# nhcha6/embodied-object-detection

Hardware: NVIDIA B200
Metric: memory write+read frames/sec (480x640, C=256) (higher is better)
Workload: dtype f32

## Files before the change

### embodied-object-detection_b200/csrc/write_mean.cu

```cuda
#include <cuda.h>
#include <stdlib.h>

#include "eod_common.cuh"
#include "tmap_cache.cuh"

namespace {

constexpr int TILE_PX = 32;

constexpr int kCountSpan = 4;

__global__ void __launch_bounds__(256) frame_count_kernel(const int32_t *__restrict__ idx, const uint8_t *__restrict__ samp,
                                                          const int32_t *__restrict__ active, int HW, int64_t n_cells,
                                                          uint32_t *__restrict__ frame_cnt, int32_t *__restrict__ slot_of_cell,
                                                          int32_t *__restrict__ slot_cell, int32_t *__restrict__ n_slots, int S)
{
    const int e = blockIdx.y;
    if (active && __ldg(active + e) <= 0) return;
    const unsigned lane = threadIdx.x & 31;
    int cellv[kCountSpan];
    bool sv[kCountSpan], validv[kCountSpan];
#pragma unroll
    for (int it = 0; it < kCountSpan; ++it) {
        const int p = (blockIdx.x * kCountSpan + it) * (int)blockDim.x + (int)threadIdx.x;
// ... 130 lines not shown
                r[h] = i < n ? (size_t)(vb * 4 + s_row[i]) * C : 0;
#pragma unroll
                for (int k = 0; k < 4; ++k)
                    if (i < n && (int)lane + 32 * k < c4) x[h][k] = reinterpret_cast<const float4 *>(sums + r[h])[lane + 32 * k];
            }
#pragma unroll
            for (int h = 0; h < 2; ++h) {
                if (i0 + 8 * h >= n) continue;
                uint2 *dst_row = reinterpret_cast<uint2 *>(norm16 + r[h]);
#pragma unroll
                for (int k = 0; k < 4; ++k) {
                    if ((int)lane + 32 * k >= c4) continue;
                    float4 y = x[h][k];
                    if (wn[h] > 1.0f) { y.x = __fdiv_rn(y.x, wn[h]); y.y = __fdiv_rn(y.y, wn[h]); y.z = __fdiv_rn(y.z, wn[h]); y.w = __fdiv_rn(y.w, wn[h]); }
                    __half2 a = __floats2half2_rn(y.x, y.y), b2 = __floats2half2_rn(y.z, y.w);
                    uint2 raw;
                    raw.x = *reinterpret_cast<uint32_t *>(&a);
                    raw.y = *reinterpret_cast<uint32_t *>(&b2);
                    dst_row[lane + 32 * k] = raw;
                }
                for (int k = lane + 128; k < c4; k += 32) {
                    float4 y = reinterpret_cast<const float4 *>(sums + r[h])[k];
                    if (wn[h] > 1.0f) { y.x = __fdiv_rn(y.x, wn[h]); y.y = __fdiv_rn(y.y, wn[h]); y.z = __fdiv_rn(y.z, wn[h]); y.w = __fdiv_rn(y.w, wn[h]); }
                    __half2 a = __floats2half2_rn(y.x, y.y), b2 = __floats2half2_rn(y.z, y.w);
                    uint2 raw;
                    raw.x = *reinterpret_cast<uint32_t *>(&a);
                    raw.y = *reinterpret_cast<uint32_t *>(&b2);
                    dst_row[k] = raw;
                }
            }
        }
        __syncthreads();
    }
}

__global__ void __launch_bounds__(256) expand_counts_kernel(const int32_t *__restrict__ idx, const uint32_t *__restrict__ frame_cnt,
                                                            int HW, int64_t n_cells, float *__restrict__ pix_n)
{
    const int e = blockIdx.y;
    const int p = blockIdx.x * blockDim.x + threadIdx.x;
    if (p >= HW) return;
    const size_t g = (size_t)e * HW + p;
    const uint32_t n = __ldg(frame_cnt + (size_t)e * n_cells + __ldg(idx + g)) & 0x7fffffffu;
    pix_n[g] = n ? __frcp_rn((float)n) : 0.f;
}

__global__ void __launch_bounds__(256) expand_counts_vec4_kernel(const int32_t *__restrict__ idx, const uint32_t *__restrict__ frame_cnt,
                                                                 int HW, int64_t n_cells, float *__restrict__ pix_n)
{
    const int e = blockIdx.y;
    const int p = (blockIdx.x * blockDim.x + threadIdx.x) * 4;
    if (p >= HW) return;
    const size_t g = (size_t)e * HW + p;
    const int4 c = __ldg(reinterpret_cast<const int4 *>(idx + g));
    const uint32_t *cnt = frame_cnt + (size_t)e * n_cells;
    const uint32_t n0 = __ldg(cnt + c.x) & 0x7fffffffu, n1 = __ldg(cnt + c.y) & 0x7fffffffu, n2 = __ldg(cnt + c.z) & 0x7fffffffu,
                   n3 = __ldg(cnt + c.w) & 0x7fffffffu;
    *reinterpret_cast<float4 *>(pix_n + g) = make_float4(n0 ? __frcp_rn((float)n0) : 0.f, n1 ? __frcp_rn((float)n1) : 0.f,
                                                         n2 ? __frcp_rn((float)n2) : 0.f, n3 ? __frcp_rn((float)n3) : 0.f);
}

__global__ void __launch_bounds__(1024) sample_mask_kernel(const uint8_t *__restrict__ observed, int HW, int stride,
                                                           uint8_t *__restrict__ samp, int32_t *__restrict__ n_sampled)
{
    __shared__ int s_warp[32];
    __shared__ int s_carry;
    const int e = blockIdx.x;
    const uint8_t *obs = observed + (size_t)e * HW;
    uint8_t *out = samp + (size_t)e * HW;
    const unsigned lane = threadIdx.x & 31, warp = threadIdx.x >> 5;
    if (threadIdx.x == 0) s_carry = 0;
    __syncthreads();
    int sampled_total = 0;
    for (int base = 0; base < HW; base += 1024) {
        const int p = base + threadIdx.x;
        const bool o = p < HW && obs[p] != 0;
        const unsigned bal = __ballot_sync(0xffffffffu, o);
        const int within = __popc(bal & ((1u << lane) - 1u));
        if (lane == 0) s_warp[warp] = __popc(bal);
        __syncthreads();
        int pre = 0;
        for (int w = 0; w < (int)warp; ++w) pre += s_warp[w];
        const int carry = s_carry;
        const int rank = carry + pre + within;
        const bool s = o && (rank % stride == 0);
        if (p < HW) out[p] = s ? 1 : 0;
        sampled_total += s ? 1 : 0;
        __syncthreads();
        if (threadIdx.x == 1023) s_carry = carry + pre + __popc(bal);
        __syncthreads();
    }
    if (n_sampled) {
        for (int o = 16; o > 0; o >>= 1) sampled_total += __shfl_xor_sync(0xffffffffu, sampled_total, o);
        if (lane == 0) s_warp[warp] = sampled_total;
        __syncthreads();
        if (threadIdx.x == 0) {
            int t = 0;
            for (int w = 0; w < 32; ++w) t += s_warp[w];
            n_sampled[e] = t;
        }
    }
}

__global__ void __launch_bounds__(1024) sample_mask_vec_kernel(const uint8_t *__restrict__ observed, int HW, int stride,
                                                               uint8_t *__restrict__ samp, int32_t *__restrict__ n_sampled)
{
    __shared__ int s_warp[2][32];
    const int e = blockIdx.x;
    const uint4 *obs = reinterpret_cast<const uint4 *>(observed + (size_t)e * HW);
    uint4 *out = reinterpret_cast<uint4 *>(samp + (size_t)e * HW);
    const unsigned lane = threadIdx.x & 31, warp = threadIdx.x >> 5;
    const int n_vec = HW >> 4;
    int carry = 0, sampled_total = 0, buf = 0;
    for (int base = 0; base < n_vec; base += 1024, buf ^= 1) {
        const int vi = base + threadIdx.x;
        uint4 q = vi < n_vec ? __ldg(obs + vi) : make_uint4(0u, 0u, 0u, 0u);
        uint32_t w[4] = {q.x, q.y, q.z, q.w};
        int cnt = 0;
#pragma unroll
        for (int k = 0; k < 4; ++k) {
            uint32_t nz = w[k] | (w[k] >> 4);
            nz |= nz >> 2;
            nz |= nz >> 1;
            w[k] = nz & 0x01010101u;
            cnt += __popc(w[k]);
        }
        int incl = cnt;
#pragma unroll
        for (int o = 1; o < 32; o <<= 1) {
            const int up = __shfl_up_sync(0xffffffffu, incl, o);
            if ((int)lane >= o) incl += up;
        }
        if (lane == 31) s_warp[buf][warp] = incl;
        __syncthreads();
        int pre = 0, total = 0;
#pragma unroll 8
        for (int x = 0; x < 32; ++x) {
            const int t = s_warp[buf][x];
            pre += x < (int)warp ? t : 0;
            total += t;
        }
        int r = (carry + pre + incl - cnt) % stride;
        carry += total;
#pragma unroll
        for (int k = 0; k < 4; ++k) {
            uint32_t o4 = 0;
#pragma unroll
            for (int b = 0; b < 4; ++b)
                if ((w[k] >> (8 * b)) & 1u) {
                    if (r == 0) { o4 |= 1u << (8 * b); ++sampled_total; }
                    if (++r == stride) r = 0;
                }
            w[k] = o4;
        }
        if (vi < n_vec) out[vi] = make_uint4(w[0], w[1], w[2], w[3]);
    }
    if (n_sampled) {
        for (int o = 16; o > 0; o >>= 1) sampled_total += __shfl_xor_sync(0xffffffffu, sampled_total, o);
        __syncthreads();
        if (lane == 0) s_warp[0][warp] = sampled_total;
        __syncthreads();
        if (threadIdx.x == 0) {
            int t = 0;
            for (int x = 0; x < 32; ++x) t += s_warp[0][x];
            n_sampled[e] = t;
        }
    }
}

__global__ void __launch_bounds__(256) box_to_image_kernel(const float *__restrict__ box_features, const uint8_t *__restrict__ masks,
                                                           int K, int C, int HW, float *__restrict__ image_features,
                                                           uint8_t *__restrict__ observed)
{
    extern __shared__ float s_feat[];
    constexpr int CH = 16;
    const int c0 = blockIdx.y * CH;
    for (int i = threadIdx.x; i < K * CH; i += blockDim.x) {
        const int k = i / CH, c = i % CH;
        s_feat[i] = (c0 + c < C) ? box_features[(size_t)k * C + c0 + c] : 0.f;
    }
    __syncthreads();
    const int p = blockIdx.x * blockDim.x + threadIdx.x;
    if (p >= HW) return;
    float acc[CH];
#pragma unroll
    for (int c = 0; c < CH; ++c) acc[c] = 0.f;
    int n = 0;
    for (int k = 0; k < K; ++k) {
        if (__ldg(masks + (size_t)k * HW + p)) {
            ++n;
#pragma unroll
            for (int c = 0; c < CH; ++c) acc[c] = __fadd_rn(acc[c], s_feat[k * CH + c]);
        }
    }
    const float fn = (float)n;
#pragma unroll
    for (int c = 0; c < CH; ++c)
        if (c0 + c < C) image_features[(size_t)(c0 + c) * HW + p] = n ? __fdiv_rn(acc[c], fn) : 0.f;
    if (blockIdx.y == 0 && observed) observed[p] = n ? 1 : 0;
}


__device__ __forceinline__ int swz(int c, int p) { return c * TILE_PX + ((((p >> 2) ^ (c & 7)) << 2) | (p & 3)); }

template <int C>
__device__ __forceinline__ void flush_runs(const float *tile, const int *s_cells, unsigned heads, unsigned samps, int pvalid,
                                           const uint32_t *__restrict__ frame_cnt_e, float *__restrict__ sums_e, int tid)
{
    constexpr int G = C / 4;
    const int nruns = __popc(heads);
    for (int item = tid; item < nruns * G; item += C) {
        const int r = item / G, g = item - r * G;
        const int p0 = __fns(heads, 0, r + 1);
        const unsigned above = heads & ~((2u << p0) - 1u);
        const int p1 = above ? (__ffs(above) - 1) : pvalid;
        const unsigned run = ((p1 >= 32) ? 0xffffffffu : ((1u << p1) - 1u)) & ~((1u << p0) - 1u);
        if (!(samps & run)) continue;
        const int cell = s_cells[p0];
        const float n = (float)(__ldg(frame_cnt_e + cell) & 0x7fffffffu);
        const int c = 4 * g;
        const float a = tile[swz(c, r)], b = tile[swz(c + 1, r)], d = tile[swz(c + 2, r)], f = tile[swz(c + 3, r)];
        red_add_v4(sums_e + (size_t)cell * C + c, __fdiv_rn(a, n), __fdiv_rn(b, n), __fdiv_rn(d, n), __fdiv_rn(f, n));
    }
}

__device__ __forceinline__ void accumulate_runs(float *tile, int c, unsigned heads, unsigned samps)
{
    float acc = 0.f;
    int r = 0;
    const float4 *row = reinterpret_cast<const float4 *>(tile + c * TILE_PX);
#pragma unroll
    for (int j = 0; j < 8; ++j) {
        const float4 v = row[j ^ (c & 7)];
        const float vv[4] = {v.x, v.y, v.z, v.w};
#pragma unroll
        for (int k = 0; k < 4; ++k) {
            const int p = 4 * j + k;
            if (p > 0 && ((heads >> p) & 1u)) {
                tile[swz(c, r)] = acc;
                ++r;
                acc = 0.f;
            }
            if ((samps >> p) & 1u) acc = __fadd_rn(acc, vv[k]);
        }
    }
    tile[swz(c, r)] = acc;
}

__device__ __forceinline__ void tile_masks(const int *s_cells, const uint8_t *s_samp, bool has_samp, int pvalid, unsigned lane,
                                           unsigned &heads, unsigned &samps)
{
    const bool valid = (int)lane < pvalid;
    const int cell = valid ? s_cells[lane] : -1;
    const int prev = __shfl_up_sync(0xffffffffu, cell, 1);
    heads = __ballot_sync(0xffffffffu, valid && (lane == 0 || prev != cell));
    samps = __ballot_sync(0xffffffffu, valid && (has_samp ? s_samp[lane] != 0 : true));
}

template <int C>
__global__ void __launch_bounds__(C) write_mean_chw_ldg_kernel(const float *__restrict__ feat, const int32_t *__restrict__ idx,
                                                               const uint8_t *__restrict__ samp, const uint32_t *__restrict__ frame_cnt,
                                                               const int32_t *__restrict__ active, int HW, int64_t n_cells, int tiles_per_ep, int n_tiles,
                                                               float *__restrict__ sums)
{
    extern __shared__ __align__(1024) unsigned char smem_raw[];
    float *tile = reinterpret_cast<float *>(smem_raw);
    int *s_cells = reinterpret_cast<int *>(tile + C * TILE_PX);
    uint8_t *s_samp = reinterpret_cast<uint8_t *>(s_cells + TILE_PX);
    const int tid = threadIdx.x, lane = tid & 31, warp = tid >> 5;
    constexpr int NW = C / 32;

    for (int t = blockIdx.x; t < n_tiles; t += gridDim.x) {
        const int e = t / tiles_per_ep, p0 = (t - e * tiles_per_ep) * TILE_PX;
        if (active && __ldg(active + e) <= 0) continue;
        const int pvalid = min(TILE_PX, HW - p0);
        const float *feat_e = feat + (size_t)e * C * HW;
#pragma unroll 4
        for (int c = warp; c < C; c += NW)
            tile[swz(c, lane)] = lane < pvalid ? __ldg(feat_e + (size_t)c * HW + p0 + lane) : 0.f;
        if (tid < TILE_PX) {
            s_cells[tid] = tid < pvalid ? __ldg(idx + (size_t)e * HW + p0 + tid) : -1;
            s_samp[tid] = (samp && tid < pvalid) ? __ldg(samp + (size_t)e * HW + p0 + tid) : 1;
        }
        __syncthreads();
        unsigned heads, samps;
        tile_masks(s_cells, s_samp, samp != nullptr, pvalid, lane, heads, samps);
        accumulate_runs(tile, tid, heads, samps);
        __syncthreads();
        flush_runs<C>(tile, s_cells, heads, samps, pvalid, frame_cnt + (size_t)e * n_cells, sums + (size_t)e * n_cells * C, tid);
        __syncthreads();
    }
}


template <int C>
struct TmaCfg {
    static constexpr int kChanBlk = C < 256 ? C : 256;
    static constexpr int kBlocks = C / kChanBlk;
    static constexpr int kJ = kChanBlk / 32;
    static constexpr int kUnitBytes = kChanBlk * TILE_PX * 4;
    static constexpr int kStages = (192 * 1024) / kUnitBytes;
    static constexpr int kThreads = 32 * (kStages + 1);
    static constexpr int kAuxCells = 0, kAuxSamp = 128, kAuxPixN = 256, kAuxUnit = 384, kAuxBytes = 512;
    static constexpr int kSmemBytes = kStages * (kUnitBytes + kAuxBytes) + 1024  + 256 ;
    static_assert(C % kChanBlk == 0 && kChanBlk % 128 == 0, "C must be 128 or a multiple of 256");
    static_assert(kSmemBytes <= 232448, "exceeds 227 KB of shared memory");
};

__device__ __forceinline__ uint64_t make_evict_first_policy()
{
    uint64_t pol;
    asm volatile("createpolicy.fractional.L2::evict_first.b64 %0, 1.0;" : "=l"(pol));
    return pol;
}

__device__ __forceinline__ void tma_load_3d_hint(uint32_t dst, const void *tmap, int x, int y, int z, uint32_t bar, uint64_t pol)
{
    asm volatile(
        "cp.async.bulk.tensor.3d.shared::cluster.global.mbarrier::complete_tx::bytes.L2::cache_hint [%0], [%1, {%2, %3, %4}], [%5], %6;" ::"r"(dst),
        "l"(tmap), "r"(x), "r"(y), "r"(z), "r"(bar), "l"(pol)
        : "memory");
}
__device__ __forceinline__ void bulk_load_1d_s(uint32_t dst, const void *src, uint32_t bytes, uint32_t bar)
{
    asm volatile("cp.async.bulk.shared::cluster.global.mbarrier::complete_tx::bytes [%0], [%1], %2, [%3];" ::"r"(dst), "l"(src), "r"(bytes), "r"(bar)
                 : "memory");
}
__device__ __forceinline__ void mbar_wait_s(uint32_t bar, uint32_t parity)
{
    asm volatile(
        "{\n\t"
        ".reg .pred p;\n\t"
        "WAIT_LOOP_S:\n\t"
        "mbarrier.try_wait.parity.shared::cta.b64 p, [%0], %1;\n\t"
        "@p bra DONE_S;\n\t"
        "bra WAIT_LOOP_S;\n\t"
        "DONE_S:\n\t"
        "}" ::"r"(bar),
        "r"(parity)
        : "memory");
}
__device__ __forceinline__ void mbar_wait_hint(uint32_t bar, uint32_t parity, uint32_t hint_ns)
{
    if (hint_ns == 0) { mbar_wait_s(bar, parity); return; }
    asm volatile(
        "{\n\t"
        ".reg .pred p;\n\t"
        "WAIT_LOOP_H:\n\t"
        "mbarrier.try_wait.parity.shared::cta.b64 p, [%0], %1, %2;\n\t"
        "@p bra DONE_H;\n\t"
        "bra WAIT_LOOP_H;\n\t"
        "DONE_H:\n\t"
        "}" ::"r"(bar),
        "r"(parity), "r"(hint_ns)
        : "memory");
}
__device__ __forceinline__ float4 lds128(uint32_t addr)
{
    float4 v;
    asm volatile("ld.shared.v4.f32 {%0, %1, %2, %3}, [%4];" : "=f"(v.x), "=f"(v.y), "=f"(v.z), "=f"(v.w) : "r"(addr));
    return v;
}
__device__ __forceinline__ uint32_t lds32(uint32_t addr)
{
    uint32_t v;
    asm volatile("ld.shared.u32 %0, [%1];" : "=r"(v) : "r"(addr));
    return v;
}
__device__ __forceinline__ void sts64(uint32_t addr, uint32_t a, uint32_t b)
{
    asm volatile("st.shared.v2.u32 [%0], {%1, %2};" ::"r"(addr), "r"(a), "r"(b) : "memory");
}
__device__ __forceinline__ uint32_t lds8(uint32_t addr)
{
    uint32_t v;
    asm volatile("ld.shared.u8 %0, [%1];" : "=r"(v) : "r"(addr));
    return v;
}

struct DetArgs {
    const int32_t *tile_off;
    float *partials;
    int32_t *run_cell;
    int32_t *status;
    int cap;
};

template <int C, bool kDry, bool kPixN, bool kDet>
__global__ void __launch_bounds__(TmaCfg<C>::kThreads, 1)
write_mean_chw_tma_kernel(const __grid_constant__ CUtensorMap tmap, const int32_t *__restrict__ idx, const uint8_t *__restrict__ samp,
                          const uint32_t *__restrict__ frame_cnt, const float *__restrict__ pix_n, const int32_t *__restrict__ active, int HW,
                          int64_t n_cells, int tiles_per_ep, int n_tiles, int group, float *__restrict__ sums, const DetArgs det,
                          int *__restrict__ work, int chunk, uint32_t wait_hint, int n_stages, int no_red)
{
    using Cfg = TmaCfg<C>;
    extern __shared__ unsigned char smem_dyn[];
    const uint32_t base = (smem_u32(smem_dyn) + 1023u) & ~1023u;
    const uint32_t aux0 = base + Cfg::kStages * Cfg::kUnitBytes;
    const uint32_t full0 = aux0 + Cfg::kStages * Cfg::kAuxBytes, empty0 = full0 + 8 * Cfg::kStages;

    const int tid = threadIdx.x;
    const int warp = tid >> 5;
    const unsigned lane = tid & 31;
    const bool has_samp = samp != nullptr;
    if (tid == 0) {
        for (int s = 0; s < Cfg::kStages; ++s) {
            asm volatile("mbarrier.init.shared::cta.b64 [%0], %1;" ::"r"(full0 + 8 * s), "r"(1));
            asm volatile("mbarrier.init.shared::cta.b64 [%0], %1;" ::"r"(empty0 + 8 * s), "r"(1));
        }
        mbar_fence_init();
        fence_proxy_async();
    }
    __syncthreads();

    const int G = (int)gridDim.x, b = (int)blockIdx.x;
    const int n_groups = n_tiles / group;
    const int units_per_group = group * Cfg::kBlocks;

    if (warp == Cfg::kStages) {
        if (lane == 0) {
            const uint64_t pol = make_evict_first_policy();
            const uint32_t tx = Cfg::kUnitBytes + TILE_PX * 4 + (has_samp ? TILE_PX : 0) + (kPixN ? TILE_PX * 4 : 0);
            int stage = 0;
            uint32_t phase = 0;
            int c = b;
            int c_next = work ? G + atomicAdd(work, 1) : c + G;
            while (c * chunk < n_groups) {
              const int c_next2 = work ? G + atomicAdd(work, 1) : c_next + G;
              const int q_end = min(n_groups, (c + 1) * chunk);
              for (int q = c * chunk; q < q_end; ++q) {
                for (int k = 0; k < units_per_group; ++k) {
                    const int cb = k / group, t = group * q + (k - cb * group);
                    const int e = t / tiles_per_ep, p0 = (t - e * tiles_per_ep) * TILE_PX;
                    const uint32_t fullb = full0 + 8 * stage, aux = aux0 + stage * Cfg::kAuxBytes;
                    mbar_wait_hint(empty0 + 8 * stage, phase ^ 1, wait_hint);
                    const bool idle = active && __ldg(active + e) <= 0;
                    sts64(aux + Cfg::kAuxUnit, (uint32_t)t, (uint32_t)cb | (idle ? 0x100u : 0u));
                    if (idle) {
                        asm volatile("mbarrier.arrive.shared::cta.b64 _, [%0];" ::"r"(fullb) : "memory");
                    } else {
                        asm volatile("mbarrier.arrive.expect_tx.shared::cta.b64 _, [%0], %1;" ::"r"(fullb), "r"(tx) : "memory");
                        tma_load_3d_hint(base + stage * Cfg::kUnitBytes, &tmap, p0, cb * Cfg::kChanBlk, e, fullb, pol);
                        bulk_load_1d_s(aux + Cfg::kAuxCells, idx + (size_t)e * HW + p0, TILE_PX * 4, fullb);
                        if (has_samp) bulk_load_1d_s(aux + Cfg::kAuxSamp, samp + (size_t)e * HW + p0, TILE_PX, fullb);
                        if (kPixN) bulk_load_1d_s(aux + Cfg::kAuxPixN, pix_n + (size_t)e * HW + p0, TILE_PX * 4, fullb);
                    }
                    if (++stage == n_stages) { stage = 0; phase ^= 1; }
                }
              }
              c = c_next;
              c_next = c_next2;
            }
            for (int s = 0; s < n_stages; ++s) {
                mbar_wait_hint(empty0 + 8 * stage, phase ^ 1, wait_hint);
                sts64(aux0 + stage * Cfg::kAuxBytes + Cfg::kAuxUnit, 0xffffffffu, 0u);
                asm volatile("mbarrier.arrive.shared::cta.b64 _, [%0];" ::"r"(full0 + 8 * stage) : "memory");
                if (++stage == n_stages) { stage = 0; phase ^= 1; }
            }
            if (work) {
                __threadfence();
                if (atomicAdd(work + 1, 1) == G - 1) {
                    work[0] = 0;
                    work[1] = 0;
                    __threadfence();
                }
            }
        }
        return;
    }

    if (warp >= n_stages) return;
    constexpr int kJ = Cfg::kJ;
    const uint32_t tile = base + warp * Cfg::kUnitBytes + lane * (TILE_PX * 4);
    const uint32_t aux = aux0 + warp * Cfg::kAuxBytes;
    const uint32_t fullb = full0 + 8 * warp, emptyb = empty0 + 8 * warp;
    const uint32_t sw = lane & 7;
    for (uint32_t phase = 0;; phase ^= 1) {
        mbar_wait_hint(fullb, phase, wait_hint);
        const int t = (int)lds32(aux + Cfg::kAuxUnit);
        if (t < 0) break;
        const uint32_t cbw = lds32(aux + Cfg::kAuxUnit + 4);
        const int cb = (int)(cbw & 0xffu);
        const bool idle = (cbw & 0x100u) != 0;
        int run_pos = kDet ? __ldg(det.tile_off + t) : 0;
        if (!kDry && !idle) {
            const int e = t / tiles_per_ep;
            const int cell = (int)lds32(aux + Cfg::kAuxCells + 4 * lane);
            const int prev = __shfl_up_sync(0xffffffffu, cell, 1);
            const unsigned grp = kDet ? 0u : __match_any_sync(0xffffffffu, cell);
            unsigned heads = __ballot_sync(0xffffffffu, kDet ? (lane == 0 || prev != cell) : ((unsigned)(__ffs(grp) - 1) == lane));
            const unsigned samps = has_samp ? __ballot_sync(0xffffffffu, lds8(aux + Cfg::kAuxSamp + lane) != 0) : 0xffffffffu;
            const float my_inv = kPixN ? __uint_as_float(lds32(aux + Cfg::kAuxPixN + 4 * lane)) : 0.f;
            float *dst = sums + ((size_t)e * n_cells) * C + cb * Cfg::kChanBlk + lane;
            const uint32_t *cnt_e = frame_cnt + (size_t)e * n_cells;

            while (heads) {
                const int p0 = __ffs(heads) - 1;
                heads &= heads - 1;
                unsigned m;
                if (kDet) {
                    const int p1 = heads ? (__ffs(heads) - 1) : TILE_PX;
                    m = samps & (0xffffffffu >> (32 - p1)) & (0xffffffffu << p0);
                } else {
                    m = samps & __shfl_sync(0xffffffffu, grp, p0);
                }
                if (m == 0) continue;
                float acc[kJ];
#pragma unroll
                for (int k = 0; k < kJ; ++k) acc[k] = 0.f;
                const int j1 = (31 - __clz(m)) >> 2;
#pragma unroll 1
                for (int j = (__ffs(m) - 1) >> 2; j <= j1; ++j) {
                    const unsigned mj = (m >> (4 * j)) & 15u;
                    if (mj == 0) continue;
                    const uint32_t a = tile + (((uint32_t)j ^ sw) << 4);
                    float4 v[kJ];
#pragma unroll
                    for (int k = 0; k < kJ; ++k) v[k] = lds128(a + k * 32 * TILE_PX * 4);
                    if (mj == 15u) {
#pragma unroll
                        for (int k = 0; k < kJ; ++k) acc[k] = __fadd_rn(__fadd_rn(__fadd_rn(__fadd_rn(acc[k], v[k].x), v[k].y), v[k].z), v[k].w);
                    } else {
                        if (mj & 1u) {
#pragma unroll
                            for (int k = 0; k < kJ; ++k) acc[k] = __fadd_rn(acc[k], v[k].x);
                        }
                        if (mj & 2u) {
#pragma unroll
                            for (int k = 0; k < kJ; ++k) acc[k] = __fadd_rn(acc[k], v[k].y);
                        }
                        if (mj & 4u) {
#pragma unroll
                            for (int k = 0; k < kJ; ++k) acc[k] = __fadd_rn(acc[k], v[k].z);
                        }
                        if (mj & 8u) {
#pragma unroll
                            for (int k = 0; k < kJ; ++k) acc[k] = __fadd_rn(acc[k], v[k].w);
                        }
                    }
                }
                const int rc = __shfl_sync(0xffffffffu, cell, p0);
                if (kDet) {
                    const int pos = run_pos++;
                    if (pos < det.cap) {
                        float *d = det.partials + ((size_t)e * det.cap + pos) * C + cb * Cfg::kChanBlk + lane;
#pragma unroll
                        for (int k = 0; k < kJ; ++k) d[32 * k] = acc[k];
                        if (cb == 0 && lane == 0) det.run_cell[(size_t)e * det.cap + pos] = rc;
                        continue;
                    }
                    if (cb == 0 && lane == 0) *det.status = 1;
                }
                float inv = __shfl_sync(0xffffffffu, my_inv, p0);
                if (!kPixN) inv = __frcp_rn((float)(__ldg(cnt_e + rc) & 0x7fffffffu));
                float *d = dst + (size_t)rc * C;
                if (no_red) continue;
#pragma unroll
                for (int k = 0; k < kJ; ++k) red_add_f32(d + 32 * k, __fmul_rn(acc[k], inv));
            }
        }
        __syncwarp();
        if (lane == 0) asm volatile("mbarrier.arrive.shared::cta.b64 _, [%0];" ::"r"(emptyb) : "memory");
    }
}

enum { FEAT_F32 = 0, FEAT_BF16 = 1, FEAT_F16 = 2 };
template <int F> struct FeatRaw { uint2 q; };
template <> struct FeatRaw<FEAT_F32> { float4 q; };
template <int F>
__device__ __forceinline__ FeatRaw<F> load_feat_raw(const void *row, int k)
{
    FeatRaw<F> r;
    if constexpr (F == FEAT_F32) r.q = ldg_stream_f4(reinterpret_cast<const float *>(row) + 4 * k);
    else asm volatile("ld.global.nc.L1::no_allocate.v2.u32 {%0, %1}, [%2];" : "=r"(r.q.x), "=r"(r.q.y) : "l"(reinterpret_cast<const uint2 *>(row) + k));
    return r;
}
template <int F>
__device__ __forceinline__ float4 widen_feat(const FeatRaw<F> &r)
{
    if constexpr (F == FEAT_F32) return r.q;
    else if constexpr (F == FEAT_BF16)
        return make_float4(__uint_as_float(r.q.x << 16), __uint_as_float(r.q.x & 0xffff0000u), __uint_as_float(r.q.y << 16), __uint_as_float(r.q.y & 0xffff0000u));
    else {
        const float2 a = __half22float2(*reinterpret_cast<const __half2 *>(&r.q.x)), b = __half22float2(*reinterpret_cast<const __half2 *>(&r.q.y));
        return make_float4(a.x, a.y, b.x, b.y);
    }
}

template <int C, int F>
__global__ void __launch_bounds__(256, 3) write_mean_hwc_kernel(const void *__restrict__ feat, const int32_t *__restrict__ idx,
                                                             const uint8_t *__restrict__ samp, const uint32_t *__restrict__ frame_cnt,
                                                             const int32_t *__restrict__ active, int HW, int64_t n_cells, int strips_per_ep,
                                                             int n_strips, float *__restrict__ sums)
{
    constexpr int V = C / 128;
    const unsigned lane = threadIdx.x & 31;
    const int warps_total = gridDim.x * (blockDim.x >> 5);
    for (int s = blockIdx.x * (blockDim.x >> 5) + (threadIdx.x >> 5); s < n_strips; s += warps_total) {
        const int e = s / strips_per_ep, p0 = (s - e * strips_per_ep) * TILE_PX;
        if (active && __ldg(active + e) <= 0) continue;
        const int pvalid = min(TILE_PX, HW - p0);
        const size_t pix0 = (size_t)e * HW + p0;
        const int my_cell = (int)lane < pvalid ? __ldg(idx + pix0 + lane) : -1;
        const bool my_s = (int)lane < pvalid && (samp ? __ldg(samp + pix0 + lane) != 0 : true);
        const unsigned samps = __ballot_sync(0xffffffffu, my_s);
        const uint32_t *cnt_e = frame_cnt + (size_t)e * n_cells;
        float *sums_e = sums + (size_t)e * n_cells * C;
        const unsigned grp = __match_any_sync(0xffffffffu, my_cell);
        unsigned leaders = __ballot_sync(0xffffffffu, (int)lane < pvalid && (unsigned)(__ffs(grp) - 1) == lane);
        constexpr int PB = (F == FEAT_F32 ? 8 : 16) / V > 0 ? (F == FEAT_F32 ? 8 : 16) / V : 1;
        while (leaders) {
            const int lead = __ffs(leaders) - 1;
            leaders &= leaders - 1;
            unsigned rem = __shfl_sync(0xffffffffu, grp, lead) & samps;
            if (rem == 0u) continue;
            const int cell = __shfl_sync(0xffffffffu, my_cell, lead);
            float4 acc[V];
#pragma unroll
            for (int v = 0; v < V; ++v) acc[v] = make_float4(0.f, 0.f, 0.f, 0.f);
#pragma unroll 1
            while (rem) {
                FeatRaw<F> raw[PB][V];
                unsigned batch = rem;
                int nb = 0;
#pragma unroll
                for (int b = 0; b < PB; ++b) {
                    if (batch) {
                        const int p = __ffs(batch) - 1;
                        batch &= batch - 1;
                        ++nb;
                        const char *row = reinterpret_cast<const char *>(feat) + (pix0 + p) * C * (F == FEAT_F32 ? 4 : 2);
#pragma unroll
                        for (int v = 0; v < V; ++v) raw[b][v] = load_feat_raw<F>(row, v * 32 + (int)lane);
                    }
                }
                rem = batch;
#pragma unroll
                for (int b = 0; b < PB; ++b) {
                    if (b < nb) {
#pragma unroll
                        for (int v = 0; v < V; ++v) {
                            const float4 f = widen_feat<F>(raw[b][v]);
                            acc[v].x = __fadd_rn(acc[v].x, f.x); acc[v].y = __fadd_rn(acc[v].y, f.y);
                            acc[v].z = __fadd_rn(acc[v].z, f.z); acc[v].w = __fadd_rn(acc[v].w, f.w);
                        }
                    }
                }
            }
            const float n = (float)(__ldg(cnt_e + cell) & 0x7fffffffu);
#pragma unroll
            for (int v = 0; v < V; ++v)
                red_add_v4(sums_e + (size_t)cell * C + v * 128 + 4 * lane, __fdiv_rn(acc[v].x, n), __fdiv_rn(acc[v].y, n), __fdiv_rn(acc[v].z, n),
                           __fdiv_rn(acc[v].w, n));
        }
    }
}

typedef CUresult (*PFN_encodeTiled)(CUtensorMap *, CUtensorMapDataType, cuuint32_t, void *, const cuuint64_t *, const cuuint64_t *,
                                    const cuuint32_t *, const cuuint32_t *, CUtensorMapInterleave, CUtensorMapSwizzle,
                                    CUtensorMapL2promotion, CUtensorMapFloatOOBfill);

PFN_encodeTiled get_encode_fn()
{
    static PFN_encodeTiled fn = nullptr;
    if (!fn) {
        void *p = nullptr;
        cudaDriverEntryPointQueryResult qres;
        if (cudaGetDriverEntryPoint("cuTensorMapEncodeTiled", &p, cudaEnableDefault, &qres) == cudaSuccess && qres == cudaDriverEntryPointSuccess)
            fn = reinterpret_cast<PFN_encodeTiled>(p);
    }
    return fn;
}

template <int C, bool kDry, bool kPixN, bool kDet = false>
int launch_tma_kernel(const CUtensorMap &tmap, const int32_t *idx, const uint8_t *samp, const uint32_t *frame_cnt, const float *pix_n,
                      const int32_t *active, int E, int HW, int64_t n_cells, float *sums, cudaStream_t st, const DetArgs det = DetArgs{})
{
    using Cfg = TmaCfg<C>;
    static unsigned long long attr_done = 0ull;
    if (int rc_attr = eod_ensure_dyn_smem(write_mean_chw_tma_kernel<C, kDry, kPixN, kDet>, Cfg::kSmemBytes, &attr_done, "eod_write_mean[tma]")) return rc_attr;
    const int tiles_per_ep = HW / TILE_PX, n_tiles = tiles_per_ep * E;
    static const int group_env = [] { const char *v = getenv("EOD_TMA_TILE_GROUP"); return v ? atoi(v) : 2; }();
    int group = (group_env == 1 || group_env == 2 || group_env == 4 || group_env == 8) ? group_env : 2;
    while (group > 1 && n_tiles % group) group >>= 1;
    const int n_groups = n_tiles / group;
    const int grid = n_groups < eod_num_sms() ? n_groups : eod_num_sms();
    static const int static_env = [] { const char *v = getenv("EOD_TMA_STATIC_TILES"); return v ? atoi(v) : 0; }();
    cudaStreamCaptureStatus cap = cudaStreamCaptureStatusNone;
    const bool capturing = cudaStreamIsCapturing(st, &cap) != cudaSuccess || cap != cudaStreamCaptureStatusNone;
    int *work = (static_env || capturing) ? nullptr : eod_work_tickets();
    static const int chunk_env = [] { const char *v = getenv("EOD_TMA_CHUNK"); return v ? atoi(v) : 8; }();
    static const int hint_env = [] { const char *v = getenv("EOD_TMA_WAIT_HINT_NS"); return v ? atoi(v) : 0; }();
    static const int stages_env = [] { const char *v = getenv("EOD_TMA_STAGES"); const int n = v ? atoi(v) : Cfg::kStages; return n >= 2 && n <= Cfg::kStages ? n : Cfg::kStages; }();
    static const int nored_env = [] { const char *v = getenv("EOD_TMA_NO_RED"); return v ? atoi(v) : 0; }();
    const int chunk = work ? (chunk_env > 0 ? chunk_env : 8) : 1;
    write_mean_chw_tma_kernel<C, kDry, kPixN, kDet><<<grid, Cfg::kThreads, Cfg::kSmemBytes, st>>>(tmap, idx, samp, frame_cnt, pix_n, active, HW, n_cells, tiles_per_ep, n_tiles, group, sums, det, work, chunk, (uint32_t)hint_env, stages_env, nored_env);
    return eod_check_launch("eod_write_mean[tma]");
}

template <int C>
int make_feature_tmap(const float *feat, int E, int HW, CUtensorMap *tmap)
{
    using Cfg = TmaCfg<C>;
    PFN_encodeTiled enc = get_encode_fn();
    EOD_REQUIRE(enc, EOD_ERR_LAUNCH, "eod_write_mean: cuTensorMapEncodeTiled entry point unavailable");
    const cuuint64_t gdim[3] = {(cuuint64_t)HW, (cuuint64_t)C, (cuuint64_t)E};
    const cuuint64_t gstr[2] = {(cuuint64_t)HW * 4, (cuuint64_t)HW * C * 4};
    const cuuint32_t box[3] = {TILE_PX, (cuuint32_t)Cfg::kChanBlk, 1};
    static const int promo_env = [] { const char *v = getenv("EOD_TMA_L2_PROMOTION"); return v ? atoi(v) : 256; }();
    const CUtensorMapL2promotion promo = promo_env == 0 ? CU_TENSOR_MAP_L2_PROMOTION_NONE
                                         : (promo_env == 128 ? CU_TENSOR_MAP_L2_PROMOTION_L2_128B : CU_TENSOR_MAP_L2_PROMOTION_L2_256B);
    const CUresult r = eod_encode_tmap_cached(enc, tmap, CU_TENSOR_MAP_DATA_TYPE_FLOAT32, 3, feat, gdim, gstr, box, promo);
    EOD_REQUIRE(r == CUDA_SUCCESS, EOD_ERR_LAUNCH, "eod_write_mean: cuTensorMapEncodeTiled failed (%d)", (int)r);
    return EOD_OK;
}

template <int C, bool kDry>
int launch_tma(const float *feat, const int32_t *idx, const uint8_t *samp, const uint32_t *frame_cnt, const float *pix_n, const int32_t *active,
               int E, int HW, int64_t n_cells, float *sums, cudaStream_t st)
{
    CUtensorMap tmap;
    const int rc = make_feature_tmap<C>(feat, E, HW, &tmap);
    if (rc) return rc;
    if (pix_n) return launch_tma_kernel<C, kDry, true>(tmap, idx, samp, frame_cnt, pix_n, active, E, HW, n_cells, sums, st);
    return launch_tma_kernel<C, kDry, false>(tmap, idx, samp, frame_cnt, nullptr, active, E, HW, n_cells, sums, st);
}

__device__ __forceinline__ void det_tile_masks(const int32_t *idx, const uint8_t *samp, size_t g0, unsigned lane, int &cell, unsigned &heads,
                                               unsigned &samps)
{
    cell = __ldg(idx + g0 + lane);
    const int prev = __shfl_up_sync(0xffffffffu, cell, 1);
    heads = __ballot_sync(0xffffffffu, lane == 0 || prev != cell);
    samps = samp ? __ballot_sync(0xffffffffu, __ldg(samp + g0 + lane) != 0) : 0xffffffffu;
}

__device__ __forceinline__ bool det_run_sampled(unsigned heads, unsigned samps, int p0)
{
    const unsigned above = heads & ~((2u << p0) - 1u);
    const int p1 = above ? (__ffs(above) - 1) : 32;
    const unsigned m = samps & (0xffffffffu >> (32 - p1)) & (0xffffffffu << p0);
    return m != 0;
}

__global__ void __launch_bounds__(256) det_tile_runs_kernel(const int32_t *__restrict__ idx, const uint8_t *__restrict__ samp, int HW,
                                                            int tiles_per_ep, int32_t *__restrict__ tile_off, int32_t *__restrict__ n_list,
                                                            int32_t *__restrict__ chunk_rows, int32_t *__restrict__ n_long)
{
    const int e = blockIdx.y, tile = blockIdx.x * 8 + (threadIdx.x >> 5);
    const unsigned lane = threadIdx.x & 31;
    if (blockIdx.x == 0 && threadIdx.x == 0) {
        n_list[e] = 0;
        chunk_rows[e] = 0;
        n_long[e] = 0;
    }
    if (tile >= tiles_per_ep) return;
    int cell;
    unsigned heads, samps;
    det_tile_masks(idx, samp, (size_t)e * HW + (size_t)tile * 32, lane, cell, heads, samps);
    const bool mine = ((heads >> lane) & 1u) && det_run_sampled(heads, samps, lane);
    const unsigned runs = __ballot_sync(0xffffffffu, mine);
    if (lane == 0) tile_off[(size_t)e * tiles_per_ep + tile] = __popc(runs);
}

__device__ void det_block_exclusive_scan(const int32_t *in, int32_t *out, int n, int32_t *total_out)
{
    __shared__ int s_warp[32];
    __shared__ int s_carry;
    const unsigned lane = threadIdx.x & 31, warp = threadIdx.x >> 5;
    if (threadIdx.x == 0) s_carry = 0;
    __syncthreads();
    for (int base = 0; base < n; base += 1024) {
        const int i = base + threadIdx.x;
        const int v = i < n ? in[i] : 0;
        int x = v;
#pragma unroll
        for (int o = 1; o < 32; o <<= 1) {
            const int y = __shfl_up_sync(0xffffffffu, x, o);
            if ((int)lane >= o) x += y;
        }
        if (lane == 31) s_warp[warp] = x;
        __syncthreads();
        if (warp == 0) {
            int w = s_warp[lane];
#pragma unroll
            for (int o = 1; o < 32; o <<= 1) {
                const int y = __shfl_up_sync(0xffffffffu, w, o);
                if ((int)lane >= o) w += y;
            }
            s_warp[lane] = w;
        }
        __syncthreads();
        const int carry = s_carry;
        const int excl = carry + (warp ? s_warp[warp - 1] : 0) + x - v;
        if (i < n) out[i] = excl;
        __syncthreads();
        if (threadIdx.x == 1023) s_carry = carry + s_warp[31];
        __syncthreads();
    }
    if (threadIdx.x == 0 && total_out) *total_out = s_carry;
}

__global__ void __launch_bounds__(1024) det_scan_tiles_kernel(int32_t *__restrict__ tile_off, int tiles_per_ep, int32_t *__restrict__ n_runs)
{
    const int e = blockIdx.x;
    det_block_exclusive_scan(tile_off + (size_t)e * tiles_per_ep, tile_off + (size_t)e * tiles_per_ep, tiles_per_ep, n_runs + e);
}

__global__ void __launch_bounds__(256) det_cell_runs_kernel(const int32_t *__restrict__ idx, const uint8_t *__restrict__ samp, int HW,
                                                            int tiles_per_ep, int64_t n_cells, const int32_t *__restrict__ tile_off, int cap,
                                                            int32_t *__restrict__ cell_runs, int32_t *__restrict__ cell_list,
                                                            int32_t *__restrict__ n_list)
{
    const int e = blockIdx.y, tile = blockIdx.x * 8 + (threadIdx.x >> 5);
    const unsigned lane = threadIdx.x & 31;
    if (tile >= tiles_per_ep) return;
    int cell;
    unsigned heads, samps;
    det_tile_masks(idx, samp, (size_t)e * HW + (size_t)tile * 32, lane, cell, heads, samps);
    const bool mine = ((heads >> lane) & 1u) && det_run_sampled(heads, samps, lane);
    const unsigned runs = __ballot_sync(0xffffffffu, mine);
    if (mine) {
        const int pos = __ldg(tile_off + (size_t)e * tiles_per_ep + tile) + __popc(runs & ((1u << lane) - 1u));
        if (pos < cap && atomicAdd(cell_runs + (size_t)e * n_cells + cell, 1) == 0)
            cell_list[(size_t)e * cap + atomicAdd(n_list + e, 1)] = cell;
    }
}

__global__ void __launch_bounds__(1024) det_scan_list_kernel(const int32_t *__restrict__ cell_runs, const int32_t *__restrict__ cell_list,
                                                             const int32_t *__restrict__ n_list, int cap, int64_t n_cells,
                                                             int32_t *__restrict__ list_off, int32_t *__restrict__ cell_off)
{
    const int e = blockIdx.x;
    const int n = __ldg(n_list + e);
    const int32_t *list = cell_list + (size_t)e * cap;
    int32_t *off = list_off + (size_t)e * cap;
    for (int i = threadIdx.x; i < n; i += 1024) off[i] = cell_runs[(size_t)e * n_cells + list[i]];
    __syncthreads();
    det_block_exclusive_scan(off, off, n, nullptr);
    __syncthreads();
    for (int i = threadIdx.x; i < n; i += 1024) cell_off[(size_t)e * n_cells + list[i]] = off[i];
}

__global__ void __launch_bounds__(256) det_claim_kernel(const int32_t *__restrict__ run_cell, const int32_t *__restrict__ n_runs, int cap,
                                                        int64_t n_cells, const int32_t *__restrict__ cell_off, int32_t *__restrict__ cell_runs,
                                                        int32_t *__restrict__ seg)
{
    const int e = blockIdx.y, pos = blockIdx.x * blockDim.x + threadIdx.x;
    if (pos >= min(__ldg(n_runs + e), cap)) return;
    const int c = __ldg(run_cell + (size_t)e * cap + pos);
    const int k = atomicSub(cell_runs + (size_t)e * n_cells + c, 1) - 1;
    seg[(size_t)e * cap + cell_off[(size_t)e * n_cells + c] + k] = pos;
}

__device__ __forceinline__ void bitonic_sort_warp(int *buf, int n2, unsigned lane)
{
    for (int size = 2; size <= n2; size <<= 1)
        for (int stride = size >> 1; stride > 0; stride >>= 1) {
            for (int q = lane; q < (n2 >> 1); q += 32) {
                const int lo = 2 * q - (q & (stride - 1)), hi = lo + stride;
                const int a = buf[lo], b = buf[hi];
                const bool asc = (lo & size) == 0;
                if ((a > b) == asc) { buf[lo] = b; buf[hi] = a; }
            }
            __syncwarp();
// ... 468 lines not shown
```

Before: 19320.

## Split TMA ring barrier so metadata arrives before feature tile

Adds a separate per-stage mbarrier for the small cell/sample/pix_n metadata loads, so consumer warps can compute run masks, heads and frame counts while the large feature tile is still in flight. It also precomputes per-run masks and prefetches the count for each head lane, and it releases the stage slot as soon as the last run's shared-memory reads finish, before the global reductions. This costs one extra barrier per stage, a little more shared memory and more barrier traffic. The early release relies on the accumulation being done before the arrive. A profiling A/B script is added as well.

After: 19670 (median of 6 runs). 1.02x the previous value.

```diff
diff --git a/embodied-object-detection_b200/csrc/write_mean.cu b/embodied-object-detection_b200/csrc/write_mean.cu
--- a/embodied-object-detection_b200/csrc/write_mean.cu
+++ b/embodied-object-detection_b200/csrc/write_mean.cu
@@ -456,7 +456,8 @@
     static constexpr int kStages = (192 * 1024) / kUnitBytes;
     static constexpr int kThreads = 32 * (kStages + 1);
     static constexpr int kAuxCells = 0, kAuxSamp = 128, kAuxPixN = 256, kAuxUnit = 384, kAuxBytes = 512;
-    static constexpr int kSmemBytes = kStages * (kUnitBytes + kAuxBytes) + 1024  + 256 ;
+    static constexpr int kBarBytes = 3 * 8 * kStages;
+    static constexpr int kSmemBytes = kStages * (kUnitBytes + kAuxBytes) + 1024  + kBarBytes;
     static_assert(C % kChanBlk == 0 && kChanBlk % 128 == 0, "C must be 128 or a multiple of 256");
     static_assert(kSmemBytes <= 232448, "exceeds 227 KB of shared memory");
 };
@@ -551,7 +552,7 @@
     extern __shared__ unsigned char smem_dyn[];
     const uint32_t base = (smem_u32(smem_dyn) + 1023u) & ~1023u;
     const uint32_t aux0 = base + Cfg::kStages * Cfg::kUnitBytes;
-    const uint32_t full0 = aux0 + Cfg::kStages * Cfg::kAuxBytes, empty0 = full0 + 8 * Cfg::kStages;
+    const uint32_t full0 = aux0 + Cfg::kStages * Cfg::kAuxBytes, empty0 = full0 + 8 * Cfg::kStages, meta0 = empty0 + 8 * Cfg::kStages;
 
     const int tid = threadIdx.x;
     const int warp = tid >> 5;
@@ -559,6 +560,7 @@
     const bool has_samp = samp != nullptr;
     if (tid == 0) {
         for (int s = 0; s < Cfg::kStages; ++s) {
+            asm volatile("mbarrier.init.shared::cta.b64 [%0], %1;" ::"r"(meta0 + 8 * s), "r"(1));
             asm volatile("mbarrier.init.shared::cta.b64 [%0], %1;" ::"r"(full0 + 8 * s), "r"(1));
             asm volatile("mbarrier.init.shared::cta.b64 [%0], %1;" ::"r"(empty0 + 8 * s), "r"(1));
         }
@@ -574,7 +576,7 @@
     if (warp == Cfg::kStages) {
         if (lane == 0) {
             const uint64_t pol = make_evict_first_policy();
-            const uint32_t tx = Cfg::kUnitBytes + TILE_PX * 4 + (has_samp ? TILE_PX : 0) + (kPixN ? TILE_PX * 4 : 0);
+            const uint32_t meta_tx = TILE_PX * 4 + (has_samp ? TILE_PX : 0) + (kPixN ? TILE_PX * 4 : 0);
             int stage = 0;
             uint32_t phase = 0;
             int c = b;
@@ -586,18 +588,20 @@
                 for (int k = 0; k < units_per_group; ++k) {
                     const int cb = k / group, t = group * q + (k - cb * group);
                     const int e = t / tiles_per_ep, p0 = (t - e * tiles_per_ep) * TILE_PX;
-                    const uint32_t fullb = full0 + 8 * stage, aux = aux0 + stage * Cfg::kAuxBytes;
+                    const uint32_t metab = meta0 + 8 * stage, fullb = full0 + 8 * stage, aux = aux0 + stage * Cfg::kAuxBytes;
                     mbar_wait_hint(empty0 + 8 * stage, phase ^ 1, wait_hint);
                     const bool idle = active && __ldg(active + e) <= 0;
                     sts64(aux + Cfg::kAuxUnit, (uint32_t)t, (uint32_t)cb | (idle ? 0x100u : 0u));
                     if (idle) {
+                        asm volatile("mbarrier.arrive.shared::cta.b64 _, [%0];" ::"r"(metab) : "memory");
                         asm volatile("mbarrier.arrive.shared::cta.b64 _, [%0];" ::"r"(fullb) : "memory");
                     } else {
-                        asm volatile("mbarrier.arrive.expect_tx.shared::cta.b64 _, [%0], %1;" ::"r"(fullb), "r"(tx) : "memory");
+                        asm volatile("mbarrier.arrive.expect_tx.shared::cta.b64 _, [%0], %1;" ::"r"(metab), "r"(meta_tx) : "memory");
+                        bulk_load_1d_s(aux + Cfg::kAuxCells, idx + (size_t)e * HW + p0, TILE_PX * 4, metab);
+                        if (has_samp) bulk_load_1d_s(aux + Cfg::kAuxSamp, samp + (size_t)e * HW + p0, TILE_PX, metab);
+                        if (kPixN) bulk_load_1d_s(aux + Cfg::kAuxPixN, pix_n + (size_t)e * HW + p0, TILE_PX * 4, metab);
+                        asm volatile("mbarrier.arrive.expect_tx.shared::cta.b64 _, [%0], %1;" ::"r"(fullb), "r"(Cfg::kUnitBytes) : "memory");
                         tma_load_3d_hint(base + stage * Cfg::kUnitBytes, &tmap, p0, cb * Cfg::kChanBlk, e, fullb, pol);
-                        bulk_load_1d_s(aux + Cfg::kAuxCells, idx + (size_t)e * HW + p0, TILE_PX * 4, fullb);
-                        if (has_samp) bulk_load_1d_s(aux + Cfg::kAuxSamp, samp + (size_t)e * HW + p0, TILE_PX, fullb);
-                        if (kPixN) bulk_load_1d_s(aux + Cfg::kAuxPixN, pix_n + (size_t)e * HW + p0, TILE_PX * 4, fullb);
                     }
                     if (++stage == n_stages) { stage = 0; phase ^= 1; }
                 }
@@ -608,6 +612,7 @@
             for (int s = 0; s < n_stages; ++s) {
                 mbar_wait_hint(empty0 + 8 * stage, phase ^ 1, wait_hint);
                 sts64(aux0 + stage * Cfg::kAuxBytes + Cfg::kAuxUnit, 0xffffffffu, 0u);
+                asm volatile("mbarrier.arrive.shared::cta.b64 _, [%0];" ::"r"(meta0 + 8 * stage) : "memory");
                 asm volatile("mbarrier.arrive.shared::cta.b64 _, [%0];" ::"r"(full0 + 8 * stage) : "memory");
                 if (++stage == n_stages) { stage = 0; phase ^= 1; }
             }
@@ -627,94 +632,108 @@
     constexpr int kJ = Cfg::kJ;
     const uint32_t tile = base + warp * Cfg::kUnitBytes + lane * (TILE_PX * 4);
     const uint32_t aux = aux0 + warp * Cfg::kAuxBytes;
-    const uint32_t fullb = full0 + 8 * warp, emptyb = empty0 + 8 * warp;
+    const uint32_t metab = meta0 + 8 * warp, fullb = full0 + 8 * warp, emptyb = empty0 + 8 * warp;
     const uint32_t sw = lane & 7;
+    auto release = [&] {
+        __syncwarp();
+        if (lane == 0) asm volatile("mbarrier.arrive.shared::cta.b64 _, [%0];" ::"r"(emptyb) : "memory");
+    };
     for (uint32_t phase = 0;; phase ^= 1) {
-        mbar_wait_hint(fullb, phase, wait_hint);
+        mbar_wait_hint(metab, phase, wait_hint);
         const int t = (int)lds32(aux + Cfg::kAuxUnit);
         if (t < 0) break;
         const uint32_t cbw = lds32(aux + Cfg::kAuxUnit + 4);
         const int cb = (int)(cbw & 0xffu);
         const bool idle = (cbw & 0x100u) != 0;
+        if (kDry || idle) {
+            mbar_wait_hint(fullb, phase, wait_hint);
+            release();
+            continue;
+        }
         int run_pos = kDet ? __ldg(det.tile_off + t) : 0;
-        if (!kDry && !idle) {
-            const int e = t / tiles_per_ep;
-            const int cell = (int)lds32(aux + Cfg::kAuxCells + 4 * lane);
+        const int e = t / tiles_per_ep;
+        const int cell = (int)lds32(aux + Cfg::kAuxCells + 4 * lane);
+        const unsigned samps = has_samp ? __ballot_sync(0xffffffffu, lds8(aux + Cfg::kAuxSamp + lane) != 0) : 0xffffffffu;
+        const float my_inv = kPixN ? __uint_as_float(lds32(aux + Cfg::kAuxPixN + 4 * lane)) : 0.f;
+        bool head;
+        unsigned mine;
+        if (kDet) {
             const int prev = __shfl_up_sync(0xffffffffu, cell, 1);
-            const unsigned grp = kDet ? 0u : __match_any_sync(0xffffffffu, cell);
-            unsigned heads = __ballot_sync(0xffffffffu, kDet ? (lane == 0 || prev != cell) : ((unsigned)(__ffs(grp) - 1) == lane));
-            const unsigned samps = has_samp ? __ballot_sync(0xffffffffu, lds8(aux + Cfg::kAuxSamp + lane) != 0) : 0xffffffffu;
-            const float my_inv = kPixN ? __uint_as_float(lds32(aux + Cfg::kAuxPixN + 4 * lane)) : 0.f;
-            float *dst = sums + ((size_t)e * n_cells) * C + cb * Cfg::kChanBlk + lane;
-            const uint32_t *cnt_e = frame_cnt + (size_t)e * n_cells;
-
-            while (heads) {
-                const int p0 = __ffs(heads) - 1;
-                heads &= heads - 1;
-                unsigned m;
-                if (kDet) {
-                    const int p1 = heads ? (__ffs(heads) - 1) : TILE_PX;
-                    m = samps & (0xffffffffu >> (32 - p1)) & (0xffffffffu << p0);
+            head = lane == 0 || prev != cell;
+            const unsigned above = __ballot_sync(0xffffffffu, head) & ~((2u << lane) - 1u);
+            mine = (above ? (above & (0u - above)) - 1u : 0xffffffffu) & ~((1u << lane) - 1u);
+        } else {
+            mine = __match_any_sync(0xffffffffu, cell);
+            head = (unsigned)(__ffs(mine) - 1) == lane;
+        }
+        mine &= samps;
+        unsigned heads = __ballot_sync(0xffffffffu, head && mine != 0u);
+        const uint32_t *cnt_e = frame_cnt + (size_t)e * n_cells;
+        uint32_t my_cnt = 0u;
+        if (!kPixN && !kDet && head && mine != 0u) my_cnt = __ldg(cnt_e + cell);
+        float *dst = sums + ((size_t)e * n_cells) * C + cb * Cfg::kChanBlk + lane;
+
+        mbar_wait_hint(fullb, phase, wait_hint);
+        if (!heads) release();
+        while (heads) {
+            const int p0 = __ffs(heads) - 1;
+            heads &= heads - 1;
+            const unsigned m = __shfl_sync(0xffffffffu, mine, p0);
+            float acc[kJ];
+#pragma unroll
+            for (int k = 0; k < kJ; ++k) acc[k] = 0.f;
+            const int j1 = (31 - __clz(m)) >> 2;
+#pragma unroll 1
+            for (int j = (__ffs(m) - 1) >> 2; j <= j1; ++j) {
+                const unsigned mj = (m >> (4 * j)) & 15u;
+                if (mj == 0) continue;
+                const uint32_t a = tile + (((uint32_t)j ^ sw) << 4);
+                float4 v[kJ];
+#pragma unroll
+                for (int k = 0; k < kJ; ++k) v[k] = lds128(a + k * 32 * TILE_PX * 4);
+                if (mj == 15u) {
+#pragma unroll
+                    for (int k = 0; k < kJ; ++k) acc[k] = __fadd_rn(__fadd_rn(__fadd_rn(__fadd_rn(acc[k], v[k].x), v[k].y), v[k].z), v[k].w);
                 } else {
-                    m = samps & __shfl_sync(0xffffffffu, grp, p0);
-                }
-                if (m == 0) continue;
-                float acc[kJ];
-#pragma unroll
-                for (int k = 0; k < kJ; ++k) acc[k] = 0.f;
-                const int j1 = (31 - __clz(m)) >> 2;
-#pragma unroll 1
-                for (int j = (__ffs(m) - 1) >> 2; j <= j1; ++j) {
-                    const unsigned mj = (m >> (4 * j)) & 15u;
-                    if (mj == 0) continue;
-                    const uint32_t a = tile + (((uint32_t)j ^ sw) << 4);
-                    float4 v[kJ];
-#pragma unroll
-                    for (int k = 0; k < kJ; ++k) v[k] = lds128(a + k * 32 * TILE_PX * 4);
-                    if (mj == 15u) {
-#pragma unroll
-                        for (int k = 0; k < kJ; ++k) acc[k] = __fadd_rn(__fadd_rn(__fadd_rn(__fadd_rn(acc[k], v[k].x), v[k].y), v[k].z), v[k].w);
-                    } else {
-                        if (mj & 1u) {
-#pragma unroll
-                            for (int k = 0; k < kJ; ++k) acc[k] = __fadd_rn(acc[k], v[k].x);
-                        }
-                        if (mj & 2u) {
-#pragma unroll
-                            for (int k = 0; k < kJ; ++k) acc[k] = __fadd_rn(acc[k], v[k].y);
-                        }
-                        if (mj & 4u) {
-#pragma unroll
-                            for (int k = 0; k < kJ; ++k) acc[k] = __fadd_rn(acc[k], v[k].z);
-                        }
-                        if (mj & 8u) {
-#pragma unroll
-                            for (int k = 0; k < kJ; ++k) acc[k] = __fadd_rn(acc[k], v[k].w);
-                        }
+                    if (mj & 1u) {
+#pragma unroll
+                        for (int k = 0; k < kJ; ++k) acc[k] = __fadd_rn(acc[k], v[k].x);
+                    }
+                    if (mj & 2u) {
+#pragma unroll
+                        for (int k = 0; k < kJ; ++k) acc[k] = __fadd_rn(acc[k], v[k].y);
+                    }
+                    if (mj & 4u) {
+#pragma unroll
+                        for (int k = 0; k < kJ; ++k) acc[k] = __fadd_rn(acc[k], v[k].z);
+                    }
+                    if (mj & 8u) {
+#pragma unroll
+                        for (int k = 0; k < kJ; ++k) acc[k] = __fadd_rn(acc[k], v[k].w);
                     }
                 }
-                const int rc = __shfl_sync(0xffffffffu, cell, p0);
-                if (kDet) {
-                    const int pos = run_pos++;
-                    if (pos < det.cap) {
-                        float *d = det.partials + ((size_t)e * det.cap + pos) * C + cb * Cfg::kChanBlk + lane;
-#pragma unroll
-                        for (int k = 0; k < kJ; ++k) d[32 * k] = acc[k];
-                        if (cb == 0 && lane == 0) det.run_cell[(size_t)e * det.cap + pos] = rc;
-                        continue;
-                    }
-                    if (cb == 0 && lane == 0) *det.status = 1;
+            }
+            if (!heads) release();
+            const int rc = __shfl_sync(0xffffffffu, cell, p0);
+            if (kDet) {
+                const int pos = run_pos++;
+                if (pos < det.cap) {
+                    float *d = det.partials + ((size_t)e * det.cap + pos) * C + cb * Cfg::kChanBlk + lane;
+#pragma unroll
+                    for (int k = 0; k < kJ; ++k) d[32 * k] = acc[k];
+                    if (cb == 0 && lane == 0) det.run_cell[(size_t)e * det.cap + pos] = rc;
+                    continue;
                 }
-                float inv = __shfl_sync(0xffffffffu, my_inv, p0);
-                if (!kPixN) inv = __frcp_rn((float)(__ldg(cnt_e + rc) & 0x7fffffffu));
-                float *d = dst + (size_t)rc * C;
-                if (no_red) continue;
-#pragma unroll
-                for (int k = 0; k < kJ; ++k) red_add_f32(d + 32 * k, __fmul_rn(acc[k], inv));
-            }
-        }
-        __syncwarp();
-        if (lane == 0) asm volatile("mbarrier.arrive.shared::cta.b64 _, [%0];" ::"r"(emptyb) : "memory");
+                if (cb == 0 && lane == 0) *det.status = 1;
+            }
+            float inv;
+            if (kPixN) inv = __shfl_sync(0xffffffffu, my_inv, p0);
+            else inv = __frcp_rn((float)((kDet ? __ldg(cnt_e + rc) : __shfl_sync(0xffffffffu, my_cnt, p0)) & 0x7fffffffu));
+            float *d = dst + (size_t)rc * C;
+            if (no_red) continue;
+#pragma unroll
+            for (int k = 0; k < kJ; ++k) red_add_f32(d + 32 * k, __fmul_rn(acc[k], inv));
+        }
     }
 }
 
diff --git a/profiles/ab_write_ring.py b/profiles/ab_write_ring.py
--- /dev/null
+++ b/profiles/ab_write_ring.py
@@ -0,0 +1,105 @@
+import argparse
+import importlib
+import json
+import math
+import os
+import subprocess
+import sys
+
+import numpy as np
+import torch
+
+sys.path.insert(0, os.path.dirname(os.path.dirname(os.path.abspath(__file__))))
+eod = importlib.import_module("embodied-object-detection_b200")
+L = eod._lib
+
+H, W = 480, 640
+
+
+def card():
+    q = "name,power.limit,clocks.sm,clocks.max.sm"
+    try:
+        out = subprocess.run(["nvidia-smi", f"--query-gpu={q}", "--format=csv,noheader", "-i", "0"], capture_output=True, text=True, timeout=30).stdout.strip()
+    except Exception as exc:
+        out = f"nvidia-smi unavailable: {exc!r}"
+    return {"device": torch.cuda.get_device_name(0), "nvidia_smi": out}
+
+
+def run(E, C, mw, mh, n_slabs, args, dev):
+    cell = np.float32(0.2)
+    eps = [eod.episodes.make_episode(1234 + e, args.frames, H, W, mw, mh, float(cell)) for e in range(E)]
+    intr = eod.compute_intrinsics(W, H, math.radians(67.5))
+    T = eod.transform3d(torch.from_numpy(np.stack([ep.xyzhe for ep in eps]).reshape(-1, 5))).reshape(E, args.frames, 4, 4)
+    pose = T[:, :, :3, :].reshape(E, args.frames, 12).permute(1, 0, 2).contiguous().to(dev)
+    depth = torch.from_numpy(np.stack([ep.depth for ep in eps])).permute(1, 0, 2, 3).contiguous().to(dev)
+    shifts = torch.from_numpy(np.stack([np.concatenate([np.zeros(3, np.float32), ep.map_world_shift]) for ep in eps])).to(dev)
+    gen = torch.Generator(device=dev).manual_seed(1234)
+    slabs = [torch.randn((E, C, H, W), device=dev, generator=gen) for _ in range(n_slabs)]
+    batch = eod.EpisodeBatch(E, mw, mh, C, H, W, dev, variant=L.WRITE_TMA, pipeline=True)
+    ev = lambda: torch.cuda.Event(enable_timing=True)
+
+    batch.project(depth[0], pose[0], shifts, intr, float(cell))
+    batch._count(None)
+    alone = {}
+    for name, variant in (("write_alone", L.WRITE_TMA), ("dry_ring", L.WRITE_TMA_DRY)):
+        batch.variant = variant
+        for i in range(3):
+            batch._write(slabs[i % n_slabs], None)
+        a, b = ev(), ev()
+        a.record()
+        for i in range(args.launches):
+            batch._write(slabs[i % n_slabs], None)
+        b.record()
+        torch.cuda.synchronize()
+        alone[name] = a.elapsed_time(b) / args.launches
+    batch.variant = L.WRITE_TMA
+    batch._finalize()
+    batch.reset()
+
+    def one_step():
+        batch.reset()
+        for t in range(args.frames):
+            batch.step(depth[t], pose[t], shifts, intr, float(cell), slabs[t % n_slabs])
+        batch.join()
+
+    for _ in range(2):
+        one_step()
+    torch.cuda.synchronize()
+    batch.profile(True)
+    a, b = ev(), ev()
+    a.record()
+    for _ in range(args.steps):
+        one_step()
+    b.record()
+    torch.cuda.synchronize()
+    stage = batch.stage_ms()
+    batch.profile(False)
+    ms_frame = a.elapsed_time(b) / (args.steps * args.frames)
+    feat_gb = E * C * H * W * 4 / 1e9
+    out = {"E": E, "C": C, "grid": [mw, mh], "frames_per_step": args.frames,
+           "write_alone_ms": round(alone["write_alone"], 4), "dry_ring_ms": round(alone["dry_ring"], 4),
+           "write_in_loop_ms": round(stage["write"], 4), "finalize_in_loop_ms": round(stage["finalize"], 4),
+           "ms_per_frame_step": round(ms_frame, 4), "frames_per_s": round(E / ms_frame * 1e3, 1),
+           "feature_GBps_alone": round(feat_gb / alone["write_alone"] * 1e3, 1), "feature_GBps_dry": round(feat_gb / alone["dry_ring"] * 1e3, 1)}
+    del batch, slabs
+    torch.cuda.empty_cache()
+    return out
+
+
+def main():
+    ap = argparse.ArgumentParser(description=__doc__.split("\n\n")[0])
+    ap.add_argument("--frames", type=int, default=4, help="frames per timed frame-step sequence")
+    ap.add_argument("--steps", type=int, default=5, help="timed sequences per setting")
+    ap.add_argument("--launches", type=int, default=20, help="timed launches of the write alone and of the dry ring")
+    args = ap.parse_args()
+    assert torch.cuda.is_available(), "needs a CUDA device"
+    dev = torch.device("cuda:0")
+    eod._lib.lib()
+    print(json.dumps({"card": card()}), flush=True)
+    print(json.dumps(run(64, 256, 500, 500, 2, args, dev)), flush=True)
+    print(json.dumps(run(32, 512, 1000, 1000, 1, args, dev)), flush=True)
+    print(json.dumps({"card_after": card()}), flush=True)
+
+
+if __name__ == "__main__":
+    main()
```
